# Jarvis73/BoxSegLiver

Hardware: AMD Instinct MI355X
Metric: CT slices/sec/node (fwd+bwd) UNet 256×256 bs=32; Dice vs ref (higher is better)
Workload: dtype f32

## Files before the change

### boxsegliver_amd/NetworksV2/UNet.py

```python
import torch

from .. import ops
from ..loss_metrics import build_head_desc, metrics_from_sums, pixel_weights
from ..utils import distribution_utils
from . import base
from .base import ModeKeys, ParamStore


def param_specs(in_channels, num_classes, init_channels, num_down_samples, normalizer, without_norm, name):
    specs = []

    def conv_unit(scope, cin, cout):
        specs.append((scope + "/weights", (3, 3, cin, cout), "conv_w"))
        if without_norm:
            specs.append((scope + "/biases", (cout,), "bias"))
        elif normalizer == "batch_norm":
            for leaf, kind in (("gamma", "gamma"), ("beta", "beta"), ("moving_mean", "moving_mean"),
                               ("moving_variance", "moving_var")):
                specs.append(("{}/BatchNorm/{}".format(scope, leaf), (cout,), kind))
        else:
            specs.append((scope + "/InstanceNorm/gamma", (cout,), "gamma"))
            specs.append((scope + "/InstanceNorm/beta", (cout,), "beta"))

    c, cin = init_channels, in_channels
# ... 33 lines not shown
        if self.params is not None:
            return
        in_ch = self.channel * (3 if getattr(self.args, "img_grad", False) else 1)
        specs = param_specs(in_ch, self.num_classes, init_channels, num_down_samples,
                            self.args.normalizer, getattr(self.args, "without_norm", False), self.name)
        self.params = ParamStore(specs, device, bias_decay=getattr(self.args, "bias_decay", False))
        self.params.initialize(self._get_initializer()[0], seed=getattr(self.args, "seed", None))

    def _net_arg_scope(self, *args, **kwargs):
        if getattr(self.args, "without_norm", False):
            self._norm = ("none", {})
        else:
            self._norm = self._get_normalization()
        return self._norm

    def _conv_unit(self, x, scope, out=None, pool=False):
        p = self.params
        kind, nparams = self._norm
        if kind == "none":
            spec = ops.NormSpec("none", 0.0, 0.0, self.is_training, self.compute_bf16)
            var = (None, p[scope + "/biases"], None, None)
        elif kind == "batch_norm":
            bn = scope + "/BatchNorm"
            spec = ops.NormSpec("batch_norm", nparams["eps"], nparams["decay"], bool(nparams["is_training"]),
                                self.compute_bf16)
            var = (p[bn + "/gamma"], p[bn + "/beta"], p[bn + "/moving_mean"], p[bn + "/moving_variance"])
        else:
            inn = scope + "/InstanceNorm"
            spec = ops.NormSpec("instance_norm", nparams["eps"], 0.0, self.is_training, self.compute_bf16)
            var = (p[inn + "/gamma"], p[inn + "/beta"], None, None)
        if pool:
            pooled, z = ops.Conv3x3NormReluPool.apply(x, p[scope + "/weights"], var[0], var[1], var[2], var[3], spec, out)
        else:
            z = ops.Conv3x3NormRelu.apply(x, p[scope + "/weights"], var[0], var[1], var[2], var[3], spec, out, None, None, None)
        if self._taps is not None:
            self._taps[scope] = z
        return (pooled, z) if pool else z

    def _build_network(self, *args, **kwargs):
        out_channels = kwargs.get("init_channels", 64)
        num_down_samples = kwargs.get("num_down_samples", 4)
        images = self._inputs["images"]
        if not images.is_cuda:
            raise ops._abi.UnetkError("UNet runs on the GPU only: move `images` to cuda (no CPU path)")
        if images.dim() != 4 or images.shape[3] != self.channel:
# ... 6 lines not shown
        nm = self.name

        if getattr(self.args, "img_grad", False):
            tensor_out = ops.image_gradients(images.to(torch.float32))
        else:
            tensor_out = images.contiguous()

        grad_mode = self.mode == ModeKeys.TRAIN
        with torch.set_grad_enabled(grad_mode):
            cats = {}
            skips = {}
            c = out_channels
            hh, ww = h, w
            for i in range(num_down_samples):
                s = "{}/Encode{}/Repeat/convolution2d_".format(nm, i + 1)
                tensor_out = self._conv_unit(tensor_out, s + "1")
                cat = torch.empty((n, hh, ww, 2 * c), dtype=self.storage_dtype, device=dev)
                skip_view = ops.alias(cat, 0, (n, hh, ww, c), cat.stride())
                tensor_out, skips[i] = self._conv_unit(tensor_out, s + "2", out=skip_view, pool=True)
                self._layers["Encode{:d}".format(i + 1)] = skips[i]
                cats[i] = cat
                c *= 2
                hh //= 2
                ww //= 2

            tensor_out = self._conv_unit(tensor_out, nm + "/ED-Bridge/ED-Bridge_1")
            tensor_out = self._conv_unit(tensor_out, nm + "/ED-Bridge/ED-Bridge_2")

            for i in reversed(range(num_down_samples)):
                c //= 2
                d = "{}/Decode{}".format(nm, i + 1)
                tensor_out = ops.DeconvConcat.apply(tensor_out, self.params[d + "/Conv2d_transpose/weights"],
                                                    self.params[d + "/Conv2d_transpose/biases"], skips[i], cats[i],
                                                    self.compute_bf16)
                tensor_out = self._conv_unit(tensor_out, d + "/Repeat/convolution2d_1")
                tensor_out = self._conv_unit(tensor_out, d + "/Repeat/convolution2d_2")

            self.ret_prob = kwargs.get("ret_prob", False)
            self.ret_pred = kwargs.get("ret_pred", False)
            labels = self._inputs.get("labels")
            if labels is not None:
                labels = labels.to(torch.int32).contiguous()
            pixel_w = pixel_weights(self.args, self._inputs, labels)
            desc = build_head_desc(self.args, n, h * w, c, self.num_classes,
                                   explicit_map=pixel_w is not None) if labels is not None else \
                ops.head_desc(n, h * w, c, self.num_classes)
            want_probs = bool(self.ret_prob or self.ret_pred or self.mode != ModeKeys.TRAIN)
            xent, dice, logits, probs, result = ops.HeadLoss.apply(
                tensor_out, self.params[nm + "/AdjustChannels/weights"], self.params[nm + "/AdjustChannels/biases"],
                labels, pixel_w, desc, want_probs)
# ... 42 lines not shown
```

### boxsegliver_amd/_abi.py

```python
import ctypes
import os
from ctypes import (POINTER, Structure, c_char_p, c_double, c_float, c_int, c_int32, c_int64, c_size_t,
                    c_void_p)

_LIB = None
LIB_PATH = os.environ.get("UNETK_LIB") or os.path.join(os.path.dirname(os.path.abspath(__file__)), "lib", "libunetk.so")

ABI_VERSION = 10
UNETK_MAX_CLASSES = 8
W_NONE, W_NUMERICAL, W_PROPORTION, W_PIXELMAP = 0, 1, 2, 3


class ConvDesc(Structure):
    _fields_ = [("N", c_int32), ("H", c_int32), ("W", c_int32), ("Cin", c_int32), ("Cout", c_int32),
                ("x_stride", c_int32), ("y_stride", c_int32), ("precision", c_int32), ("dilation", c_int32)]


FP32, BF16, BF16S = 0, 1, 2


class DeconvDesc(Structure):
    _fields_ = [("N", c_int32), ("H", c_int32), ("W", c_int32), ("Cin", c_int32), ("Cout", c_int32),
                ("out_stride", c_int32), ("out_coff", c_int32), ("precision", c_int32)]

# ... 30 lines not shown
class LitsGuideDesc(Structure):
    _fields_ = [("N", c_int32), ("H", c_int32), ("W", c_int32), ("C", c_int32), ("src_h", c_int32), ("src_w", c_int32),
                ("n_obj", c_int32), ("min_std", c_float)]


P = c_void_p
_SIGNATURES = {
    "unetk_lits_batch": (c_int, [POINTER(LitsDesc), c_void_p, c_void_p, c_void_p, c_void_p, c_void_p, c_void_p, c_void_p]),
    "unetk_lits_spatial_guide": (c_int, [POINTER(LitsGuideDesc), P, P, P, P, P]),
    "unetk_lits_context": (c_int, [P, c_int64, c_int, P, c_int, c_int, P, P, P, P]),
    "unetk_abi_version": (c_int, []),
    "unetk_nan_watch": (c_int, [P, P, c_int32, P]),
    "unetk_png_unfilter": (c_int, [P, c_int64, c_int, c_int, c_int, c_int, P, c_int64, P, P]),
    "unetk_conv3x3_fwd_affine_ok": (c_int, [POINTER(ConvDesc), c_int]),
    "unetk_conv3x3_fwd_affine": (c_int, [POINTER(ConvDesc), P, P, P, P, P, P, c_int, P, c_size_t, P]),
    "unetk_prof_reset": (c_int, [c_int]),
    "unetk_prof_enable": (c_int, [c_int]),
    "unetk_prof_mark": (c_int, []),
    "unetk_prof_read": (c_int, [c_int, c_int, POINTER(c_float)]),
    "unetk_prof_name": (c_int, [c_int, ctypes.c_char_p, c_int]),
    "unetk_error_string": (c_char_p, [c_int]),
    "unetk_conv3x3_pack": (c_int, [P, c_int, c_int, P, P, P]),
    "unetk_pack_item_blocks": (c_int, [c_int, c_int, c_int]),
    "unetk_pack_many": (c_int, [P, c_int, c_int, P]),
    "unetk_conv3x3_pack_bf16": (c_int, [P, c_int, c_int, P, P, P]),
    "unetk_conv3x3_pack_bf16s": (c_int, [P, c_int, c_int, P, P, P]),
    "unetk_conv3x3_stat_rows": (c_int, [POINTER(ConvDesc)]),
    "unetk_conv3x3_fwd": (c_int, [POINTER(ConvDesc), P, P, P, P, P]),
    "unetk_conv3x3_dgrad": (c_int, [POINTER(ConvDesc), P, P, P, P]),
    "unetk_conv3x3_ws_bytes": (c_size_t, [POINTER(ConvDesc)]),
# ... 136 lines not shown
```

### boxsegliver_amd/csrc/common.h

```cpp
#pragma once
#include <hip/hip_ext.h>
#include <hip/hip_runtime.h>
#include <stdint.h>

#include "unetk.h"

extern int g_unetk_prof_on;
void unetk_prof_pair(const void* fn, hipEvent_t* a, hipEvent_t* b);
#define UNETK_LAUNCH(kern, grid, block, lds, st, ...)                                                   \
  do {                                                                                                  \
    if (__builtin_expect(g_unetk_prof_on, 0)) {                                                         \
      hipEvent_t pa_, pb_;                                                                              \
      unetk_prof_pair(reinterpret_cast<const void*>(kern), &pa_, &pb_);                                 \
      hipExtLaunchKernelGGL(kern, grid, block, lds, st, pa_, pb_, 0, __VA_ARGS__);                      \
    } else {                                                                                            \
      hipLaunchKernelGGL(kern, grid, block, lds, st, __VA_ARGS__);                                      \
    }                                                                                                   \
  } while (0)

typedef float f32x16 __attribute__((ext_vector_type(16)));

#define UNETK_LAUNCH_CHECK()                      \
  do {                                            \
    hipError_t e_ = hipGetLastError();            \
// ... 97 lines not shown
  int stride;
  int Hin, Win, pbh, pbw;
  int ntaps[4], tap_off[4][4], tap_panel[4][4];
  int ooh[4], oow[4];
  int os, Hd, Wd;
  int dil;
  int kd, dshift0, dstep;
  int dsd, din;
  int64_t dplane;
  const void* ny;
  const float *nsc, *nsh, *nmu, *nrs;
  int nys, nsst;
  const float *asc, *ash;
  void* pool;
  int pool_s;
  float* sk_slab;
  size_t sk_slab_bytes;
  int sk_tiles, sk_nc, sk_maxp, sk_whole;
  int ng;
  int g_chan[12], g_dz[12], g_ntaps[12], g_off[12][4], g_panel[12][4];
  int dpar;
  int64_t dpar_yoff;
  int nlive;
  unsigned khalf;
  int klive[32];
};
inline int unetk_live_chunks(const uint32_t live8[2], int K) {
  const uint64_t m = (uint64_t)live8[0] | ((uint64_t)live8[1] << 32);
  if (m == 0 || K % 16 != 0 || K > 512) return K / 16;
  int n = 0;
// ... 78 lines not shown
```

### boxsegliver_amd/csrc/conv_igemm.hip

```cpp
#include "common.h"

#include <type_traits>
#include "pack.h"

namespace {

__device__ __attribute__((aligned(16))) float kZeroF4[4] = {};

constexpr int CK = 16;
#ifndef HALO_LD_T
#define HALO_LD_T 2
#endif
#ifndef HALO_ST_T
#define HALO_ST_T 7
#endif
constexpr int PS = 20;
constexpr int TW = 16;

#ifndef UNETK_HALO_ROWPAD
#define UNETK_HALO_ROWPAD 1
#endif
constexpr int halo_row_f(int S, int DIL) {
  return (S == 1 && DIL == 1 && UNETK_HALO_ROWPAD) ? ((S * TW + 2 * DIL) * PS + 63) / 64 * 64 : (S * TW + 2 * DIL) * PS;
}

template <int WM, int WN, int TM, int TN, int S = 1, int DIL = 1, int MODE = 0>
__global__ __launch_bounds__(WM* WN * 64, (TM * TN == 8 ? 2 : 1)) void conv3x3_igemm_kernel(ConvParams p) {
  constexpr bool NBR = MODE == 2, ACC = MODE == 1, AFF = MODE >= 3, POOL = MODE == 4;
  static_assert(!AFF || (S == 1 && DIL == 1), "the fused inference epilogue is for plain 3x3 convs");
  static_assert(S == 1 || DIL == 1, "strided atrous convs are not needed");
  static_assert(!NBR || (S == 1 && DIL == 1), "the fused reduction is for plain 3x3 convs");
  constexpr int NT = WM * WN * 64;
  constexpr int BM = WM * TM * 32, BN = WN * TN * 32;
  constexpr int TH = BM / TW, HH = S * TH + 2 * DIL;
  constexpr int HWD = S * TW + 2 * DIL;
  constexpr int HALO_PIX = HH * HWD;
  constexpr int HROW = halo_row_f(S, DIL);
  constexpr int HALO_F = HH * HROW;
  constexpr int WB_F = CK * BN;
  constexpr int HR = (HALO_PIX * 4 + NT - 1) / NT;
  constexpr int WR = (CK / 4 * BN + NT - 1) / NT;
  constexpr int WF4 = CK / 4 * BN;
  constexpr bool W_ALL = WF4 == WR * NT;

  extern __shared__ __attribute__((aligned(16))) float smem[];
  float* halo = smem;
  float* wbuf = smem + 2 * HALO_F;
// ... 5 lines not shown
  const int l31 = lane & 31, h = lane >> 5;

  const int bid = xcd_remap(blockIdx.x, gridDim.x);
  const int ntile = bid % p.n_ntiles;
  const int mtile = bid / p.n_ntiles;
  const int tw_i = mtile % p.tiles_w;
  const int th_i = (mtile / p.tiles_w) % p.tiles_h;
  const int n_img = mtile / (p.tiles_w * p.tiles_h);
  const int h0 = th_i * TH, w0 = tw_i * TW, n0 = ntile * BN;

  const int64_t ximg = p.xa.off(n_img), yimg = p.ya.off(n_img);

  int64_t hoff[HR];
  bool hok[HR];
  int hlds[HR];
#pragma unroll
  for (int r = 0; r < HR; ++r) {
    const int idx = tid + r * NT;
    const int pix = idx >> 2, q = idx & 3;
    const int hh = pix / HWD, ww = pix - hh * HWD;
    const int gh = S * h0 - (S == 1 ? DIL : p.pbh) + hh, gw = S * w0 - (S == 1 ? DIL : p.pbw) + ww;
    const int Hin = S == 1 ? p.H : p.Hin, Win = S == 1 ? p.W : p.Win;
    hok[r] = (idx < HALO_PIX * 4) && gh >= 0 && gh < Hin && gw >= 0 && gw < Win;
    hoff[r] = ximg + ((int64_t)gh * Win + gw) * p.xs + q * 4;
    hlds[r] = (idx < HALO_PIX * 4) ? hh * HROW + ww * PS + q * 4 : -1;
  }
  const int cin4 = p.Cin >> 2;
  int64_t woff[WR];
#pragma unroll
  for (int r = 0; r < WR; ++r) {
    const int idx = min(tid + r * NT, WF4 - 1);
    const int q = idx / BN, n = idx - q * BN;
    woff[r] = ((int64_t)q * p.Cout + n0 + n) * 4;
  }

  const int nchunks = p.Cin / CK;
  int c_begin = 0, c_end = nchunks;
  if (p.kd > 1) {
    const int dep = n_img % p.spg;
    int dt_lo = 0, dt_hi = p.kd;
    while (dt_lo < dt_hi && dep * p.dsd + p.dshift0 + dt_lo < 0) ++dt_lo;
    while (dt_hi > dt_lo && dep * p.dsd + p.dshift0 + dt_hi - 1 >= p.din) --dt_hi;
    c_begin = dt_lo * nchunks;
    c_end = dt_hi * nchunks;
  }
  float4 hreg[HR], wreg[WR];
  auto load_halo = [&](int cc) {
    const int dt = p.kd > 1 ? cc / nchunks : 0, c = cc - dt * nchunks;
    const int64_t soff = (p.kd > 1 ? (int64_t)(p.dshift0 + dt) * p.dplane : 0) + c * CK;
#pragma unroll
    for (int r = 0; r < HR; ++r) hreg[r] = ldg4(hok[r] ? p.x + hoff[r] + soff : kZeroF4);
  };
  auto store_halo = [&](int buf) {
#pragma unroll
    for (int r = 0; r < HR; ++r)
      if (hlds[r] >= 0) *reinterpret_cast<float4*>(&halo[buf * HALO_F + hlds[r]]) = hreg[r];
  };
  auto load_w = [&](int cc, int t) {
    const int dt = p.kd > 1 ? cc / nchunks : 0, c = cc - dt * nchunks;
    const float* base = p.wp + ((int64_t)(dt * 9 + t) * cin4 + c * (CK / 4)) * p.Cout * 4;
#pragma unroll
    for (int r = 0; r < WR; ++r)
      wreg[r] = ldg4(base + woff[r]);
  };
  auto store_w = [&](int buf) {
#pragma unroll
    for (int r = 0; r < WR; ++r)
      if (W_ALL || tid + r * NT < WF4) *reinterpret_cast<float4*>(&wbuf[buf * WB_F + (tid + r * NT) * 4]) = wreg[r];
// ... 5 lines not shown
    const int sub = wm * TM + tm;
    abase[tm] = S * (2 * sub + (l31 >> 4)) * HROW + S * (l31 & 15) * PS + 4 * h;
  }
  const int bbase = (h * BN + wn * TN * 32 + l31) * 4;

  f32x16 acc[TM][TN];
#pragma unroll
  for (int tm = 0; tm < TM; ++tm)
#pragma unroll
    for (int tn = 0; tn < TN; ++tn)
#pragma unroll
      for (int r = 0; r < 16; ++r) acc[tm][tn][r] = 0.f;

  load_halo(c_begin);
  load_w(c_begin, 0);
  store_halo(0);
  store_w(0);
  __syncthreads();

  int step = 0;
  for (int c = c_begin; c < c_end; ++c) {
    const float* hb = halo + ((c - c_begin) & 1) * HALO_F;
    const bool more_chunks = (c + 1 < c_end);
#pragma unroll
    for (int t = 0; t < 9; ++t, ++step) {
      const bool has_next = (t < 8) || more_chunks;
      if (has_next) load_w(t < 8 ? c : c + 1, t < 8 ? t + 1 : 0);
      if (t == HALO_LD_T && more_chunks) load_halo(c + 1);
      __builtin_amdgcn_sched_barrier(0);

      const float* wb = wbuf + (step & 1) * WB_F;
      const int toff = (t / 3) * DIL * HROW + (t % 3) * DIL * PS;
#pragma unroll
      for (int g = 0; g < CK / 8; ++g) {
        float4 a[TM], b[TN];
#pragma unroll
        for (int tm = 0; tm < TM; ++tm)
          a[tm] = *reinterpret_cast<const float4*>(&hb[abase[tm] + toff + 8 * g]);
#pragma unroll
        for (int tn = 0; tn < TN; ++tn)
          b[tn] = *reinterpret_cast<const float4*>(&wb[bbase + (2 * g * BN + tn * 32) * 4]);
#pragma unroll
        for (int tm = 0; tm < TM; ++tm)
#pragma unroll
          for (int tn = 0; tn < TN; ++tn) {
            acc[tm][tn] = __builtin_amdgcn_mfma_f32_32x32x2f32(a[tm].x, b[tn].x, acc[tm][tn], 0, 0, 0);
            acc[tm][tn] = __builtin_amdgcn_mfma_f32_32x32x2f32(a[tm].y, b[tn].y, acc[tm][tn], 0, 0, 0);
            acc[tm][tn] = __builtin_amdgcn_mfma_f32_32x32x2f32(a[tm].z, b[tn].z, acc[tm][tn], 0, 0, 0);
            acc[tm][tn] = __builtin_amdgcn_mfma_f32_32x32x2f32(a[tm].w, b[tn].w, acc[tm][tn], 0, 0, 0);
          }
      }

      if (has_next) store_w((step + 1) & 1);
      if (t == HALO_ST_T && more_chunks) store_halo((c + 1 - c_begin) & 1);
      __syncthreads();
    }
  }

  float ssum[TN], ssq[TN];
#pragma unroll
  for (int tn = 0; tn < TN; ++tn) ssum[tn] = ssq[tn] = 0.f;
  float nsc[TN], nsh[TN], nmu[TN], nrs[TN];
  if constexpr (NBR) {
#pragma unroll
    for (int tn = 0; tn < TN; ++tn) {
      const int64_t o = (int64_t)n_img * p.nsst + n0 + (wn * TN + tn) * 32 + l31;
      nsc[tn] = p.nsc[o]; nsh[tn] = p.nsh[o]; nmu[tn] = p.nmu[o]; nrs[tn] = p.nrs[o];
    }
  }
// ... 372 lines not shown
  static bool attr_done = false;
  if (!attr_done) {
    hipError_t e = hipFuncSetAttribute((const void*)kern, hipFuncAttributeMaxDynamicSharedMemorySize, (int)lds);
    if (e != hipSuccess) return (int)e;
    attr_done = true;
  }
  const int grid = n_mtiles * p.n_ntiles;
  UNETK_LAUNCH(kern, dim3(grid), dim3(WM * WN * 64), lds, st, p);
  UNETK_LAUNCH_CHECK();
  return UNETK_OK;
}

template <int WM, int WN, int TM, int TN, int S = 1, int DIL = 1, bool NBR = false>
int launch_igemm(const ConvParams& p, int n_mtiles, hipStream_t st) {
  if constexpr (NBR) return launch_igemm_mode<WM, WN, TM, TN, S, DIL, 2>(p, n_mtiles, st);
  if (p.asc != nullptr) {
    if constexpr (S == 1 && DIL == 1) {
      if (p.accumulate || p.stat != nullptr) return UNETK_E_UNSUPPORTED;
      return p.pool != nullptr ? launch_igemm_mode<WM, WN, TM, TN, 1, 1, 4>(p, n_mtiles, st)
                               : launch_igemm_mode<WM, WN, TM, TN, 1, 1, 3>(p, n_mtiles, st);
    } else {
      return UNETK_E_UNSUPPORTED;
    }
  }
  if (p.accumulate) return launch_igemm_mode<WM, WN, TM, TN, S, DIL, 1>(p, n_mtiles, st);
  return launch_igemm_mode<WM, WN, TM, TN, S, DIL, 0>(p, n_mtiles, st);
}

}

static int s2_th(int Cout) { return Cout % 128 == 0 ? 4 : 8; }
int unetk_conv_stat_rows(int N, int H, int W, int Cin, int Cout, int spg, int stride, int dil) {
  if (dil == 2) return N * ((H + 7) / 8) * ((W + TW - 1) / TW);
  if (stride == 2) return N * ((H + s2_th(Cout) - 1) / s2_th(Cout)) * ((W + TW - 1) / TW);
  if (unetk_conv_lin_ok(N, H, W, Cin, Cout, spg)) return unetk_conv_stat_rows_lin(N, H, W, spg, Cout);
  const int th = tile_rows(N, H, W, Cin, Cout, spg, false);
  return N * ((H + th - 1) / th) * ((W + TW - 1) / TW);
}

bool unetk_conv_stride2_ok(int Cin, int Cout) { return Cin % CK == 0 && Cout % 64 == 0; }

int unetk_conv_run(ConvParams p, hipStream_t st) {
  if ((p.ny != nullptr || p.asc != nullptr) && (p.stride == 2 || p.dil == 2)) return UNETK_E_UNSUPPORTED;
  if (p.stride == 2) {
    if (p.bf16 || !unetk_conv_stride2_ok(p.Cin, p.Cout) || p.xs % 4 != 0) return UNETK_E_UNSUPPORTED;
    p.tiles_h = (p.H + s2_th(p.Cout) - 1) / s2_th(p.Cout);
    p.tiles_w = (p.W + TW - 1) / TW;
    const int n_mt = p.N * p.tiles_h * p.tiles_w;
    p.stat_rows = n_mt;
    if (p.Cout % 128 == 0) {
      p.n_ntiles = p.Cout / 128;
      return launch_igemm<2, 2, 1, 2, 2>(p, n_mt, st);
    }
    p.n_ntiles = p.Cout / 64;
    return launch_igemm<4, 1, 1, 2, 2>(p, n_mt, st);
  }
  if (p.dil == 2) {
    if (p.bf16 || p.Cin % CK != 0 || p.Cout % 64 != 0 || p.xs % 4 != 0) return UNETK_E_UNSUPPORTED;
// ... 190 lines not shown
  ConvParams p{};
  if (d->precision == UNETK_BF16S) {
    if (unetk_conv_bf16_ok(d->Cin, d->Cout)) p.bf16 = UNETK_BF16S;
    else p.ybf16 = 1;
  }
  p.x = (const float*)x; p.wp = (const float*)w; p.y = (float*)z; p.stat = nullptr;
  p.asc = scale; p.ash = shift; p.pool = pooled; p.pool_s = pooled_stride;
  if (ws && unetk_aligned16(ws) && ws_bytes > 0) { p.sk_slab = (float*)ws; p.sk_slab_bytes = ws_bytes; }
  p.dil = d->dilation;
  p.N = d->N; p.H = d->H; p.W = d->W; p.Cin = d->Cin; p.Cout = d->Cout; p.xs = d->x_stride; p.ys = d->y_stride;
  p.xa = unetk_dense_addr(p.H, p.W, p.xs);
  p.ya = unetk_dense_addr(p.H, p.W, p.ys);
  return unetk_conv_run(p, (hipStream_t)stream);
}

extern "C" int unetk_conv3x3_dgrad(const unetk_conv_desc* d, const void* dy, const void* w, void* dx,
                                   void* stream) {
  return unetk_conv3x3_dgrad_ws(d, dy, w, dx, nullptr, 0, stream);
}

extern "C" int unetk_conv3x3_dgrad_ws(const unetk_conv_desc* d, const void* dy, const void* w, void* dx, void* ws,
                                      size_t ws_bytes, void* stream) {
  UNETK_REQUIRE(conv_desc_ok(d) && dy && w && dx);
  UNETK_REQUIRE(unetk_aligned16(dy) && unetk_aligned16(w) && unetk_aligned16(dx));
  if (pick_cfg(d->Cout, d->Cin).id < 0) return UNETK_E_UNSUPPORTED;
  UNETK_REQUIRE(d->x_stride % 4 == 0 && d->y_stride % 4 == 0);
  if (d->precision != UNETK_FP32 && !unetk_conv_bf16_ok(d->Cout, d->Cin)) return UNETK_E_UNSUPPORTED;
  if (d->precision == UNETK_BF16S && d->dilation > 1) return UNETK_E_UNSUPPORTED;
  ConvParams p{};
  p.bf16 = d->precision;
// ... 44 lines not shown
```

### boxsegliver_amd/ops.py

```python
import ctypes
import os

import torch

from . import _abi
from ._abi import Conv3dDesc, ConvDesc, Deconv3dDesc, DeconvDesc, HeadDesc, NormDesc, check, ptr, stream_ptr


class _Workspace(object):

    def __init__(self):
        self._bufs = {}

    def get(self, nbytes, device):
        nbytes = max(int(nbytes), 16)
        key = (device.type, device.index)
        buf = self._bufs.get(key)
        if buf is None or buf.numel() < nbytes:
            buf = torch.empty(int(nbytes * 1.25) + 256, dtype=torch.uint8, device=device)
            self._bufs[key] = buf
        return buf


WORKSPACE = _Workspace()
FUSE_EVAL = os.environ.get("UNETK_FUSE_EVAL", "1") != "0"
FUSE_NBR = True
FUSED_NBR = {}
DEBUG_CAPTURE = None
PROFILE_SHAPES = False
PROFILE = None


PACK_BATCH = True
PARAM_GEN = 0
_PARAM_FLATS = {}


def register_param_buffer(flat):
    import weakref
    _PARAM_FLATS[flat.untyped_storage().data_ptr()] = weakref.ref(flat)

# ... 131 lines not shown


def _timed(tag_fn, flops, fmt=None, args=(), nbytes_fn=None):
    if PROFILE is None:
        return _NO_TIMER
    tag = tag_fn() if callable(tag_fn) else tag_fn
    return _Timed(tag, flops, fmt.format(*args) if fmt else None, nbytes_fn(tag) if nbytes_fn else 0)


def _timed_hbm(tag, t, passes, extra=0):
    if PROFILE is None:
        return _NO_TIMER
    return _Timed(tag, 0.0, None, t.numel() * t.element_size() * passes + extra)


def _igemm_tag(cin, cout, bf16=False, h=0, n=1 << 20, w=1 << 10, nbr=False):
    def cdiv(a, b):
        return -(-a // b)

    def big(bn):
        return h % 16 == 0 and not (nbr and cin < 256) and n * (h // 16) * cdiv(w, 16) * (cout // bn) >= 512
    if bf16 and cin % 32 == 0 and cout % 32 == 0:
        bs = ",true>" if int(bf16) == _abi.BF16S else ">"
        if int(bf16) == _abi.BF16S and h >= 24 and (cout % 128 == 0 or cout == 64):
            bn = 128 if cout % 128 == 0 else 64
            if n * cdiv(h, 32) * cdiv(w, 16) * (cout // bn) >= 200:
                return "conv3x3_bf16s_kernel<{}{}>".format(bn // 16, ",nbr" if nbr else "")
        if cout % 128 == 0:
            tall = h >= 24 and n * cdiv(h, 32) * cdiv(w, 16) * (cout // 128) >= 200
            return ("conv3x3_igemm_bf16_kernel<4,2,4,2" if tall else "conv3x3_igemm_bf16_kernel<2,2,2,2") + bs
        if cout % 64 == 0:
# ... 202 lines not shown
                      "conv3x3_pack_bf16")
            kind, perm = PK_CONV_BF16, 1 if prec == _abi.BF16S else 0
        else:
            wp_f = torch.empty(9 * cin * cout, dtype=torch.float32, device=w.device)
            wp_d = torch.empty_like(wp_f) if want_dgrad else None
            check(_abi.lib().unetk_conv3x3_pack(ptr(w), cin, cout, ptr(wp_f), ptr(wp_d), stream_ptr()), "conv3x3_pack")
            kind, perm = PK_CONV_F32, 0
        return wp_f, wp_d, [(kind, perm, cin, cout, w.data_ptr(), wp_f.data_ptr(), wp_d.data_ptr() if want_dgrad else None)]
    return PACKS.get(w, ("c3", prec, bool(want_dgrad)), build)


def conv_uses_mfma(cin, cout):
    return cin % 16 == 0 and cout % 32 == 0


def conv3x3_fwd(x, w, cout, want_stats=True, y=None, bf16=False, dilation=1):
    _require_cuda(x, w)
    n, h, wd, cin = x.shape
    prec = precision_of(bf16)
    if y is None:
        y = torch.empty((n, h, wd, cout), dtype=storage_dtype(prec), device=x.device)
    if prec == _abi.BF16S:
        assert y.dtype == torch.bfloat16 and x.dtype == (torch.bfloat16 if conv_uses_mfma(cin, cout) else torch.float32), \
            (x.dtype, y.dtype, cin, cout)
    else:
        assert x.dtype == torch.float32 and y.dtype == torch.float32
    d = ConvDesc(n, h, wd, cin, cout, _pix_stride(x), _pix_stride(y), prec, int(dilation))
    stats = None
    rows = 0
    if want_stats:
        rows = _abi.lib().unetk_conv3x3_stat_rows(ctypes.byref(d))
        if rows <= 0:
            check(rows, "conv3x3_stat_rows")
        stats = torch.empty((2, rows, cout), dtype=torch.float32, device=x.device)
    nws = _abi.lib().unetk_conv3x3_ws_bytes(ctypes.byref(d)) if prec == _abi.FP32 else 0
    ws = WORKSPACE.get(nws, x.device) if nws else None
    with _timed(lambda: _igemm_tag(cin, cout, bf16, h, n, wd), 18.0 * n * h * wd * cin * cout, "fwd {}x{}x{} {}->{}", (n, h, wd, cin, cout),
                lambda tag: (x.numel() * x.element_size() + y.numel() * y.element_size()) if tag in ("conv3x3_direct_kernel", "conv3x3_c3_mfma_kernel") else 0):
        check(_abi.lib().unetk_conv3x3_fwd_ws(ctypes.byref(d), ptr(x), ptr(w), ptr(y), ptr(stats), ptr(ws), nws,
                                              stream_ptr()), "conv3x3_fwd")
    return y, stats, rows


def conv3x3_fwd_affine(x, w, cout, scale, shift, z=None, pool=False, bf16=False):
    _require_cuda(x, w)
    n, h, wd, cin = x.shape
    prec = precision_of(bf16)
    if z is None:
        z = torch.empty((n, h, wd, cout), dtype=storage_dtype(prec), device=x.device)
    d = ConvDesc(n, h, wd, cin, cout, _pix_stride(x), _pix_stride(z), prec, 1)
    pooled = torch.empty((n, h // 2, wd // 2, cout), dtype=z.dtype, device=x.device) if pool else None
# ... 928 lines not shown
    check(_abi.lib().unetk_norm_se_bwd_add(ctypes.byref(d), ptr(y), ptr(dy), ptr(aff[0]), ptr(aff[1]), ptr(aff[2]),
                                           ptr(a_mat.contiguous()), ptr(k2.contiguous()), stream_ptr()), "norm_se_bwd_add")
    return dy


class NormSpec(object):

    def __init__(self, kind="batch_norm", eps=1e-3, decay=0.999, training=True, bf16=False):
        assert kind in ("batch_norm", "instance_norm", "none")
        self.kind, self.eps, self.decay, self.training = kind, eps, decay, training
        self.guide_leaky = False
        self.guide_alpha = 0.2
        self.guide_per_sample = False
        self.guide_post = False
        self.dropout = None
        self.se = None
        self.bf16 = precision_of(bf16)

    @property
    def per_sample(self):
        return self.kind == "instance_norm"


class Conv3x3NormRelu(_Op):

    @staticmethod
    def forward(ctx, x, w, gamma, beta, moving_mean, moving_var, spec, out, guide, gw, gb, den=None, dilation=1, se_feat=None):
        _require_cuda(x, w)
        cin, cout = w.shape[2], w.shape[3]
        dilation = int(dilation or 1)
        if dilation != 1 and (bool(getattr(spec, "bf16", False)) or not conv_uses_mfma(cin, cout)):
            raise _abi.UnetkError("atrous conv (rate {}) needs the fp32 MFMA path (Cin % 16, Cout % 64)".format(dilation))
        if den is not None:
            den = den.contiguous()
        mfma = conv_uses_mfma(cin, cout)
        prec = precision_of(getattr(spec, "bf16", 0))
        bf16 = prec if conv_uses_bf16(cin, cout) else 0
        if prec == _abi.BF16S:
            if mfma and (cin % 64 or cout % 64):
                raise _abi.UnetkError("bf16 storage needs Cin % 64 == 0 and Cout % 64 == 0 (got {}->{})".format(cin, cout))
            bf16 = prec
        need_dx = ctx.needs_input_grad[0]
        if mfma:
            wp_f, wp_d = conv3x3_pack(w, want_dgrad=need_dx, bf16=bf16)
        else:
            wp_f, wp_d = w, None
            if need_dx:
                raise _abi.UnetkError("conv3x3 input gradient needs Cin%64==0 and Cout%16==0 "
                                      "(got {}->{})".format(cin, cout))
        plain = spec.kind == "none"
        se = getattr(spec, "se", None)
        use_batch_stats = (spec.training or spec.per_sample) and not plain
        if se is not None and (plain or den is not None):
            raise _abi.UnetkError("--use_se needs a normalised unit and no other density gain")
        fprec = precision_of(bf16)
        if FUSE_EVAL and not spec.training and not use_batch_stats and se is None and den is None and guide is None \
                and gb is None and fprec in (_abi.FP32, _abi.BF16S) and dilation == 1:
# ... 6 lines not shown
                nd = norm_desc((n_, h_, w_, cout), False, _pix_stride(z), 0, 0, 0)
                if plain:
                    sc, sh = torch.ones_like(beta), beta.detach().contiguous()
                else:
                    aff = norm_finalize(nd, None, 0, gamma, beta, spec.eps, spec.decay, False, moving_mean, moving_var, x.device)
                    sc, sh = aff[2], aff[3]
                pooled = torch.empty((n_, h_ // 2, w_ // 2, cout), dtype=z.dtype, device=x.device) if with_pool else None
                tag = _igemm_tag(cin, cout, bf16, h_, n_, w_) + ("+affine+relu+pool" if with_pool else "+affine+relu")
                nws = _abi.lib().unetk_conv3x3_ws_bytes(ctypes.byref(fd))
                ws = WORKSPACE.get(nws, x.device) if nws else None
                with _timed(tag, 18.0 * n_ * h_ * w_ * cin * cout, "infer {}x{}x{} {}->{}", (n_, h_, w_, cin, cout)):
                    check(_abi.lib().unetk_conv3x3_fwd_affine(ctypes.byref(fd), ptr(x), ptr(wp_f), ptr(sc), ptr(sh), ptr(z),
                                                              ptr(pooled), cout, ptr(ws), nws, stream_ptr()), "conv3x3_fwd_affine")
                ctx.pooled = pooled
                return alias(z) if out is not None else z
        y, stats, rows = conv3x3_fwd(x, wp_f, cout, want_stats=use_batch_stats or se is not None, bf16=bf16, dilation=dilation)
        z = out if out is not None else torch.empty_like(y)
        g_ch = 0 if guide is None else guide.shape[-1]
        if g_ch:
            gw = gw.contiguous()
        if gb is not None:
            gb = gb.contiguous()
        d = norm_desc(y.shape, spec.per_sample, _pix_stride(z), g_ch, cout if g_ch else 0, 0)
        if g_ch and getattr(spec, "guide_leaky", False):
            alpha = float(getattr(spec, "guide_alpha", 0.2))
            d.guide_leaky = 1 if alpha == 0.2 else 2
            d.guide_alpha = alpha
        if g_ch and getattr(spec, "guide_post", False):
            d.guide_leaky = 3
        if getattr(spec, "guide_per_sample", False):
            d.guide_per_sample = 1
# ... 21 lines not shown
                mean_b = norm_finalize(ps, stats, rows, None, None, spec.eps, 0.0, True, None, None, y.device)[0]
                xhat_mean = ((mean_b - aff[0]) * aff[1]).detach()
            with torch.enable_grad():
                g_leaf = gamma.detach().requires_grad_(True) if gamma is not None else None
                b_leaf = beta.detach().requires_grad_(True) if beta is not None else None
                pooled = xhat_mean if g_leaf is None else xhat_mean * g_leaf
                if b_leaf is not None:
                    pooled = pooled + (b_leaf if m_mean is None else m_mean * b_leaf)
                pooled = pooled + torch.zeros_like(xhat_mean).requires_grad_(True) if not pooled.requires_grad else pooled
                pooled.retain_grad()
                f_leaf = se_feat.detach().requires_grad_(True) if se_feat is not None else None
                gains = se(pooled, f_leaf)
            den = gains.detach().contiguous()
            se_graph = (g_leaf, b_leaf, pooled, gains, xhat_mean, f_leaf, m_mean)
        ctx.pooled = None
        if getattr(ctx, "want_pool", False) and POOL_FUSED and se is None and den is None and g_ch == 0 and gb is None \
                and d.dropout_keep == 0 and y.shape[1] % 2 == 0 and y.shape[2] % 2 == 0:
            ctx.pooled = norm_apply_relu_pool(d, y, aff, z)
        else:
            norm_apply_relu(d, y, aff, z, guide, gw, gb, den)
        simple = (not plain and se is None and den is None and g_ch == 0 and gb is None and d.dropout_keep == 0)
        if spec.training:
            src = getattr(x, "_unetk_unit", None)
            ctx.producer = src if (need_dx and src is not None and dilation == 1) else None
            ctx.simple = simple
            if getattr(ctx, "want_pool", False):
                ctx.unit_saved = (x, y, aff, guide, gw, gb, den)
            else:
                ctx.save_for_backward(x, y, aff, guide, gw, gb, den)
            ctx.se_graph = se_graph
            ctx.wp_d = wp_d
            ctx.need_dx = need_dx
            ctx.bf16 = bf16
            ctx.dilation = dilation
            ctx.desc = d
            ctx.has = (gamma is not None, beta is not None)
            ctx.sinks = (grad_sink(w, ctx), grad_sink(gamma, ctx) if se is None else None, grad_sink(beta, ctx) if se is None and not plain else None)
            ctx.w_dbg = w.detach() if DEBUG_CAPTURE is not None else None
            ctx.gb_dbg = (gamma, beta) if DEBUG_CAPTURE is not None else None
            ctx.z_dbg = z.detach() if DEBUG_CAPTURE is not None else None
        zr = alias(z) if out is not None else z
        if spec.training and simple and out is None:
            zr._unetk_unit = (y, aff, spec.per_sample)
        return zr

    @staticmethod
    def backward(ctx, dz):
        return Conv3x3NormRelu._backward(ctx, dz)

    @staticmethod
    def _backward(ctx, dz, pool=None):
        x, y, aff, guide, gw, gb, den = ctx.saved_tensors[:7]
        pre = None
        if pool is None:
            pre = FUSED_NBR.pop(dz.data_ptr(), None) if DEBUG_CAPTURE is None else None
            if pre is not None and not (ctx.simple and pre[0] == y.data_ptr() and pre[1] == tuple(dz.shape) and dz.is_contiguous()
                                        and pre[4] == dz._version):
                pre = None
# ... 419 lines not shown
```

### include/unetk.h

```cpp
#ifndef UNETK_H_
#define UNETK_H_

#include <stddef.h>
#include <stdint.h>

#ifdef __cplusplus
extern "C" {
#endif

#define UNETK_OK 0
#define UNETK_E_BADARG (-1)
#define UNETK_E_UNSUPPORTED (-2)
#define UNETK_E_WORKSPACE (-3)

#define UNETK_MAX_CLASSES 8

#define UNETK_W_NONE 0
#define UNETK_W_NUMERICAL 1
#define UNETK_W_PROPORTION 2
#define UNETK_W_PIXELMAP 3

#define UNETK_LOSS_XENTROPY 1
#define UNETK_LOSS_DICE 2

// ... 40 lines not shown
                      float* stat_partials, void* stream);

int unetk_conv3x3_dgrad(const unetk_conv_desc* d, const void* dy, const void* w, void* dx,
                        void* stream);

size_t unetk_conv3x3_ws_bytes(const unetk_conv_desc* d);
int unetk_conv3x3_fwd_ws(const unetk_conv_desc* d, const void* x, const void* w, void* y, float* stat_partials,
                         void* ws, size_t ws_bytes, void* stream);
int unetk_conv3x3_dgrad_ws(const unetk_conv_desc* d, const void* dy, const void* w, void* dx, void* ws,
                           size_t ws_bytes, void* stream);

int unetk_conv3x3_fwd_affine_ok(const unetk_conv_desc* d, int with_pool);
int unetk_conv3x3_fwd_affine(const unetk_conv_desc* d, const void* x, const void* w, const float* scale,
                             const float* shift, void* z, void* pooled, int pooled_stride, void* ws, size_t ws_bytes,
                             void* stream);

int unetk_conv3x3_dgrad_nbr_rows(const unetk_conv_desc* d);
int unetk_conv3x3_dgrad_nbr(const unetk_conv_desc* d, const void* dy, const void* w, void* dx, const void* prod_y,
                            int prod_y_stride, const float* scale, const float* shift, const float* mean,
                            const float* rstd, int per_sample, float* partials, void* stream);

size_t unetk_conv3x3_wgrad_ws_bytes(const unetk_conv_desc* d);
int unetk_conv3x3_wgrad(const unetk_conv_desc* d, const void* x, const void* dy, float* dw,
                        void* ws, size_t ws_bytes, void* stream);

typedef struct unetk_conv3d_desc {
  int32_t N, D, H, W, Cin, Cout;
  int32_t kd;
  int32_t sd;
  int32_t shw;
// ... 252 lines not shown
```

Before: 437.5.

## Fold norm+ReLU of first conv into next conv's halo loader

```diff
diff --git a/boxsegliver_amd/NetworksV2/UNet.py b/boxsegliver_amd/NetworksV2/UNet.py
--- a/boxsegliver_amd/NetworksV2/UNet.py
+++ b/boxsegliver_amd/NetworksV2/UNet.py
@@ -71,7 +71,7 @@
             self._norm = self._get_normalization()
         return self._norm
 
-    def _conv_unit(self, x, scope, out=None, pool=False):
+    def _conv_unit(self, x, scope, out=None, pool=False, defer=False):
         p = self.params
         kind, nparams = self._norm
         if kind == "none":
@@ -86,6 +86,7 @@
             inn = scope + "/InstanceNorm"
             spec = ops.NormSpec("instance_norm", nparams["eps"], 0.0, self.is_training, self.compute_bf16)
             var = (p[inn + "/gamma"], p[inn + "/beta"], None, None)
+        spec.defer_apply = bool(defer) and not pool and self._taps is None
         if pool:
             pooled, z = ops.Conv3x3NormReluPool.apply(x, p[scope + "/weights"], var[0], var[1], var[2], var[3], spec, out)
         else:
@@ -122,7 +123,7 @@
             hh, ww = h, w
             for i in range(num_down_samples):
                 s = "{}/Encode{}/Repeat/convolution2d_".format(nm, i + 1)
-                tensor_out = self._conv_unit(tensor_out, s + "1")
+                tensor_out = self._conv_unit(tensor_out, s + "1", defer=True)
                 cat = torch.empty((n, hh, ww, 2 * c), dtype=self.storage_dtype, device=dev)
                 skip_view = ops.alias(cat, 0, (n, hh, ww, c), cat.stride())
                 tensor_out, skips[i] = self._conv_unit(tensor_out, s + "2", out=skip_view, pool=True)
@@ -132,7 +133,7 @@
                 hh //= 2
                 ww //= 2
 
-            tensor_out = self._conv_unit(tensor_out, nm + "/ED-Bridge/ED-Bridge_1")
+            tensor_out = self._conv_unit(tensor_out, nm + "/ED-Bridge/ED-Bridge_1", defer=True)
             tensor_out = self._conv_unit(tensor_out, nm + "/ED-Bridge/ED-Bridge_2")
 
             for i in reversed(range(num_down_samples)):
@@ -141,7 +142,7 @@
                 tensor_out = ops.DeconvConcat.apply(tensor_out, self.params[d + "/Conv2d_transpose/weights"],
                                                     self.params[d + "/Conv2d_transpose/biases"], skips[i], cats[i],
                                                     self.compute_bf16)
-                tensor_out = self._conv_unit(tensor_out, d + "/Repeat/convolution2d_1")
+                tensor_out = self._conv_unit(tensor_out, d + "/Repeat/convolution2d_1", defer=True)
                 tensor_out = self._conv_unit(tensor_out, d + "/Repeat/convolution2d_2")
 
             self.ret_prob = kwargs.get("ret_prob", False)
diff --git a/boxsegliver_amd/_abi.py b/boxsegliver_amd/_abi.py
--- a/boxsegliver_amd/_abi.py
+++ b/boxsegliver_amd/_abi.py
@@ -68,6 +68,8 @@
     "unetk_png_unfilter": (c_int, [P, c_int64, c_int, c_int, c_int, c_int, P, c_int64, P, P]),
     "unetk_conv3x3_fwd_affine_ok": (c_int, [POINTER(ConvDesc), c_int]),
     "unetk_conv3x3_fwd_affine": (c_int, [POINTER(ConvDesc), P, P, P, P, P, P, c_int, P, c_size_t, P]),
+    "unetk_conv3x3_fwd_apply_ok": (c_int, [POINTER(ConvDesc)]),
+    "unetk_conv3x3_fwd_apply": (c_int, [POINTER(ConvDesc), P, P, P, c_int, P, P, P, P, P]),
     "unetk_prof_reset": (c_int, [c_int]),
     "unetk_prof_enable": (c_int, [c_int]),
     "unetk_prof_mark": (c_int, []),
diff --git a/boxsegliver_amd/csrc/common.h b/boxsegliver_amd/csrc/common.h
--- a/boxsegliver_amd/csrc/common.h
+++ b/boxsegliver_amd/csrc/common.h
@@ -135,6 +135,9 @@
   const float *asc, *ash;
   void* pool;
   int pool_s;
+  const float *lsc, *lsh;
+  float* lz;
+  int lsst;
   float* sk_slab;
   size_t sk_slab_bytes;
   int sk_tiles, sk_nc, sk_maxp, sk_whole;
diff --git a/boxsegliver_amd/csrc/conv_igemm.hip b/boxsegliver_amd/csrc/conv_igemm.hip
--- a/boxsegliver_amd/csrc/conv_igemm.hip
+++ b/boxsegliver_amd/csrc/conv_igemm.hip
@@ -26,11 +26,13 @@
 
 template <int WM, int WN, int TM, int TN, int S = 1, int DIL = 1, int MODE = 0>
 __global__ __launch_bounds__(WM* WN * 64, (TM * TN == 8 ? 2 : 1)) void conv3x3_igemm_kernel(ConvParams p) {
-  constexpr bool NBR = MODE == 2, ACC = MODE == 1, AFF = MODE >= 3, POOL = MODE == 4;
+  constexpr bool NBR = MODE == 2, ACC = MODE == 1, AFF = MODE == 3 || MODE == 4, POOL = MODE == 4, APL = MODE == 5;
+  static_assert(!APL || (S == 1 && DIL == 1), "the normaliser in the loader is for plain 3x3 convs");
   static_assert(!AFF || (S == 1 && DIL == 1), "the fused inference epilogue is for plain 3x3 convs");
   static_assert(S == 1 || DIL == 1, "strided atrous convs are not needed");
   static_assert(!NBR || (S == 1 && DIL == 1), "the fused reduction is for plain 3x3 convs");
   constexpr int NT = WM * WN * 64;
+  static_assert(NT % 4 == 0, "a thread's halo slots share one channel quad");
   constexpr int BM = WM * TM * 32, BN = WN * TN * 32;
   constexpr int TH = BM / TW, HH = S * TH + 2 * DIL;
   constexpr int HWD = S * TW + 2 * DIL;
@@ -66,6 +68,7 @@
   int64_t hoff[HR];
   bool hok[HR];
   int hlds[HR];
+  bool hzo[APL ? HR : 1];
 #pragma unroll
   for (int r = 0; r < HR; ++r) {
     const int idx = tid + r * NT;
@@ -76,6 +79,7 @@
     hok[r] = (idx < HALO_PIX * 4) && gh >= 0 && gh < Hin && gw >= 0 && gw < Win;
     hoff[r] = ximg + ((int64_t)gh * Win + gw) * p.xs + q * 4;
     hlds[r] = (idx < HALO_PIX * 4) ? hh * HROW + ww * PS + q * 4 : -1;
+    if constexpr (APL) hzo[r] = hok[r] && ntile == 0 && hh >= DIL && hh < HH - DIL && ww >= DIL && ww < HWD - DIL;
   }
   const int cin4 = p.Cin >> 2;
   int64_t woff[WR];
@@ -97,13 +101,40 @@
     c_end = dt_hi * nchunks;
   }
   float4 hreg[HR], wreg[WR];
+  float4 lsc = make_float4(0.f, 0.f, 0.f, 0.f), lsh = lsc;
+  const float* lsc_p = nullptr;
+  const float* lsh_p = nullptr;
+  if constexpr (APL) {
+    lsc_p = p.lsc + (int64_t)n_img * p.lsst + (tid & 3) * 4;
+    lsh_p = p.lsh + (int64_t)n_img * p.lsst + (tid & 3) * 4;
+  }
   auto load_halo = [&](int cc) {
     const int dt = p.kd > 1 ? cc / nchunks : 0, c = cc - dt * nchunks;
     const int64_t soff = (p.kd > 1 ? (int64_t)(p.dshift0 + dt) * p.dplane : 0) + c * CK;
 #pragma unroll
     for (int r = 0; r < HR; ++r) hreg[r] = ldg4(hok[r] ? p.x + hoff[r] + soff : kZeroF4);
+    if constexpr (APL) {
+      lsc = ldg4(lsc_p + c * CK);
+      lsh = ldg4(lsh_p + c * CK);
+    }
   };
-  auto store_halo = [&](int buf) {
+  auto store_halo = [&](int buf, int cc) {
+    if constexpr (APL) {
+      const float4 sh = make_float4(lsh.x + 0.f, lsh.y + 0.f, lsh.z + 0.f, lsh.w + 0.f);
+#pragma unroll
+      for (int r = 0; r < HR; ++r) {
+        float4 u;
+        u.x = fmaxf(fmaf(hreg[r].x, lsc.x, sh.x), 0.f); u.y = fmaxf(fmaf(hreg[r].y, lsc.y, sh.y), 0.f);
+        u.z = fmaxf(fmaf(hreg[r].z, lsc.z, sh.z), 0.f); u.w = fmaxf(fmaf(hreg[r].w, lsc.w, sh.w), 0.f);
+        if (!hok[r]) u = make_float4(0.f, 0.f, 0.f, 0.f);
+        hreg[r] = u;
+        if (hlds[r] >= 0) *reinterpret_cast<float4*>(&halo[buf * HALO_F + hlds[r]]) = u;
+      }
+#pragma unroll
+      for (int r = 0; r < HR; ++r)
+        if (hzo[r]) stg4(p.lz + hoff[r] + cc * CK, hreg[r]);
+      return;
+    }
 #pragma unroll
     for (int r = 0; r < HR; ++r)
       if (hlds[r] >= 0) *reinterpret_cast<float4*>(&halo[buf * HALO_F + hlds[r]]) = hreg[r];
@@ -139,7 +170,7 @@
 
   load_halo(c_begin);
   load_w(c_begin, 0);
-  store_halo(0);
+  store_halo(0, c_begin);
   store_w(0);
   __syncthreads();
 
@@ -149,8 +180,8 @@
     const bool more_chunks = (c + 1 < c_end);
 #pragma unroll
     for (int t = 0; t < 9; ++t, ++step) {
-      const bool has_next = (t < 8) || more_chunks;
-      if (has_next) load_w(t < 8 ? c : c + 1, t < 8 ? t + 1 : 0);
+      const bool has_next = APL || (t < 8) || more_chunks;
+      if (has_next) load_w((t < 8 || !more_chunks) ? c : c + 1, t < 8 ? t + 1 : 0);
       if (t == HALO_LD_T && more_chunks) load_halo(c + 1);
       __builtin_amdgcn_sched_barrier(0);
 
@@ -176,8 +207,9 @@
           }
       }
 
+      if constexpr (APL) __builtin_amdgcn_sched_barrier(0);
       if (has_next) store_w((step + 1) & 1);
-      if (t == HALO_ST_T && more_chunks) store_halo((c + 1 - c_begin) & 1);
+      if (t == HALO_ST_T && more_chunks) store_halo((c + 1 - c_begin) & 1, c + 1);
       __syncthreads();
     }
   }
@@ -580,6 +612,14 @@
 template <int WM, int WN, int TM, int TN, int S = 1, int DIL = 1, bool NBR = false>
 int launch_igemm(const ConvParams& p, int n_mtiles, hipStream_t st) {
   if constexpr (NBR) return launch_igemm_mode<WM, WN, TM, TN, S, DIL, 2>(p, n_mtiles, st);
+  if (p.lz != nullptr) {
+    if constexpr (S == 1 && DIL == 1) {
+      if (p.accumulate || p.asc != nullptr || p.kd > 1) return UNETK_E_UNSUPPORTED;
+      return launch_igemm_mode<WM, WN, TM, TN, 1, 1, 5>(p, n_mtiles, st);
+    } else {
+      return UNETK_E_UNSUPPORTED;
+    }
+  }
   if (p.asc != nullptr) {
     if constexpr (S == 1 && DIL == 1) {
       if (p.accumulate || p.stat != nullptr) return UNETK_E_UNSUPPORTED;
@@ -607,7 +647,10 @@
 bool unetk_conv_stride2_ok(int Cin, int Cout) { return Cin % CK == 0 && Cout % 64 == 0; }
 
 int unetk_conv_run(ConvParams p, hipStream_t st) {
-  if ((p.ny != nullptr || p.asc != nullptr) && (p.stride == 2 || p.dil == 2)) return UNETK_E_UNSUPPORTED;
+  if ((p.ny != nullptr || p.asc != nullptr || p.lz != nullptr) && (p.stride == 2 || p.dil == 2)) return UNETK_E_UNSUPPORTED;
+  if (p.lz != nullptr && (p.bf16 || p.ny != nullptr || pick_cfg(p.Cin, p.Cout).id < 0 ||
+                          unetk_conv_lin_ok(p.N, p.H, p.W, p.Cin, p.Cout, p.spg < 1 ? 1 : p.spg)))
+    return UNETK_E_UNSUPPORTED;
   if (p.stride == 2) {
     if (p.bf16 || !unetk_conv_stride2_ok(p.Cin, p.Cout) || p.xs % 4 != 0) return UNETK_E_UNSUPPORTED;
     p.tiles_h = (p.H + s2_th(p.Cout) - 1) / s2_th(p.Cout);
@@ -828,6 +871,29 @@
   return unetk_conv_run(p, (hipStream_t)stream);
 }
 
+extern "C" int unetk_conv3x3_fwd_apply_ok(const unetk_conv_desc* d) {
+  if (!conv_desc_ok(d) || d->dilation > 1 || d->precision != UNETK_FP32) return 0;
+  if (pick_cfg(d->Cin, d->Cout).id < 0 || d->x_stride != d->Cin || d->y_stride % 4 != 0) return 0;
+  return unetk_conv_lin_ok(d->N, d->H, d->W, d->Cin, d->Cout, 1) ? 0 : 1;
+}
+
+extern "C" int unetk_conv3x3_fwd_apply(const unetk_conv_desc* d, const void* prod_y, const float* scale, const float* shift,
+                                       int per_sample, void* z, const void* w, void* y, float* stat_partials,
+                                       void* stream) {
+  UNETK_REQUIRE(conv_desc_ok(d) && prod_y && scale && shift && z && w && y);
+  UNETK_REQUIRE(unetk_aligned16(prod_y) && unetk_aligned16(z) && unetk_aligned16(w) && unetk_aligned16(y));
+  UNETK_REQUIRE(unetk_aligned16(scale) && unetk_aligned16(shift));
+  if (!unetk_conv3x3_fwd_apply_ok(d)) return UNETK_E_UNSUPPORTED;
+  ConvParams p{};
+  p.x = (const float*)prod_y; p.wp = (const float*)w; p.y = (float*)y; p.stat = stat_partials;
+  p.lsc = scale; p.lsh = shift; p.lz = (float*)z; p.lsst = per_sample ? d->Cin : 0;
+  p.dil = d->dilation;
+  p.N = d->N; p.H = d->H; p.W = d->W; p.Cin = d->Cin; p.Cout = d->Cout; p.xs = d->x_stride; p.ys = d->y_stride;
+  p.xa = unetk_dense_addr(p.H, p.W, p.xs);
+  p.ya = unetk_dense_addr(p.H, p.W, p.ys);
+  return unetk_conv_run(p, (hipStream_t)stream);
+}
+
 extern "C" int unetk_conv3x3_dgrad(const unetk_conv_desc* d, const void* dy, const void* w, void* dx,
                                    void* stream) {
   return unetk_conv3x3_dgrad_ws(d, dy, w, dx, nullptr, 0, stream);
diff --git a/boxsegliver_amd/ops.py b/boxsegliver_amd/ops.py
--- a/boxsegliver_amd/ops.py
+++ b/boxsegliver_amd/ops.py
@@ -25,6 +25,7 @@
 WORKSPACE = _Workspace()
 FUSE_EVAL = os.environ.get("UNETK_FUSE_EVAL", "1") != "0"
 FUSE_NBR = True
+APPLY_IN_LOADER = os.environ.get("UNETK_APPLY_IN_LOADER", "1") != "0"
 FUSED_NBR = {}
 DEBUG_CAPTURE = None
 PROFILE_SHAPES = False
@@ -186,7 +187,9 @@
     return _Timed(tag, 0.0, None, t.numel() * t.element_size() * passes + extra)
 
 
-def _igemm_tag(cin, cout, bf16=False, h=0, n=1 << 20, w=1 << 10, nbr=False):
+def _igemm_tag(cin, cout, bf16=False, h=0, n=1 << 20, w=1 << 10, nbr=False, apply=False):
+    if apply:
+        return _igemm_tag(cin, cout, bf16, h, n, w, nbr) + "+apply"
     def cdiv(a, b):
         return -(-a // b)
 
@@ -419,7 +422,24 @@
     return cin % 16 == 0 and cout % 32 == 0
 
 
-def conv3x3_fwd(x, w, cout, want_stats=True, y=None, bf16=False, dilation=1):
+def conv3x3_fwd_apply_ok(x, cout, bf16=False, dilation=1):
+    n, h, wd, cin = x.shape
+    if precision_of(bf16) != _abi.FP32 or int(dilation) != 1 or x.dtype != torch.float32 or not x.is_contiguous():
+        return False
+    d = ConvDesc(n, h, wd, cin, cout, cin, cout, _abi.FP32, 1)
+    return _abi.lib().unetk_conv3x3_fwd_apply_ok(ctypes.byref(d)) == 1
+
+
+def materialize(z):
+    pend = getattr(z, "_unetk_deferred", None)
+    if pend is not None:
+        z._unetk_deferred = None
+        py, paff, _, nd = pend
+        norm_apply_relu(nd, py, paff, z)
+    return z
+
+
+def conv3x3_fwd(x, w, cout, want_stats=True, y=None, bf16=False, dilation=1, deferred=None):
     _require_cuda(x, w)
     n, h, wd, cin = x.shape
     prec = precision_of(bf16)
@@ -440,6 +460,14 @@
         stats = torch.empty((2, rows, cout), dtype=torch.float32, device=x.device)
     nws = _abi.lib().unetk_conv3x3_ws_bytes(ctypes.byref(d)) if prec == _abi.FP32 else 0
     ws = WORKSPACE.get(nws, x.device) if nws else None
+    if deferred is not None:
+        py, paff, per_sample = deferred[0], deferred[1], deferred[2]
+        assert py.is_contiguous() and x.is_contiguous() and tuple(py.shape) == tuple(x.shape) and py.dtype == x.dtype == torch.float32
+        with _timed(lambda: _igemm_tag(cin, cout, bf16, h, n, wd, apply=True), 18.0 * n * h * wd * cin * cout, "fwd+apply {}x{}x{} {}->{}",
+                    (n, h, wd, cin, cout)):
+            check(_abi.lib().unetk_conv3x3_fwd_apply(ctypes.byref(d), ptr(py), ptr(paff[2]), ptr(paff[3]), 1 if per_sample else 0,
+                                                     ptr(x), ptr(w), ptr(y), ptr(stats), stream_ptr()), "conv3x3_fwd_apply")
+        return y, stats, rows
     with _timed(lambda: _igemm_tag(cin, cout, bf16, h, n, wd), 18.0 * n * h * wd * cin * cout, "fwd {}x{}x{} {}->{}", (n, h, wd, cin, cout),
                 lambda tag: (x.numel() * x.element_size() + y.numel() * y.element_size()) if tag in ("conv3x3_direct_kernel", "conv3x3_c3_mfma_kernel") else 0):
         check(_abi.lib().unetk_conv3x3_fwd_ws(ctypes.byref(d), ptr(x), ptr(w), ptr(y), ptr(stats), ptr(ws), nws,
@@ -1398,6 +1426,7 @@
         self.guide_per_sample = False
         self.guide_post = False
         self.dropout = None
+        self.defer_apply = False
         self.se = None
         self.bf16 = precision_of(bf16)
 
@@ -1425,6 +1454,13 @@
                 raise _abi.UnetkError("bf16 storage needs Cin % 64 == 0 and Cout % 64 == 0 (got {}->{})".format(cin, cout))
             bf16 = prec
         need_dx = ctx.needs_input_grad[0]
+        deferred = getattr(x, "_unetk_deferred", None)
+        if deferred is not None:
+            if APPLY_IN_LOADER and spec.training and mfma and not bf16 and conv3x3_fwd_apply_ok(x, cout, bf16, dilation):
+                x._unetk_deferred = None
+            else:
+                materialize(x)
+                deferred = None
         if mfma:
             wp_f, wp_d = conv3x3_pack(w, want_dgrad=need_dx, bf16=bf16)
         else:
@@ -1461,7 +1497,8 @@
                                                               ptr(pooled), cout, ptr(ws), nws, stream_ptr()), "conv3x3_fwd_affine")
                 ctx.pooled = pooled
                 return alias(z) if out is not None else z
-        y, stats, rows = conv3x3_fwd(x, wp_f, cout, want_stats=use_batch_stats or se is not None, bf16=bf16, dilation=dilation)
+        y, stats, rows = conv3x3_fwd(x, wp_f, cout, want_stats=use_batch_stats or se is not None, bf16=bf16, dilation=dilation,
+                                     deferred=deferred)
         z = out if out is not None else torch.empty_like(y)
         g_ch = 0 if guide is None else guide.shape[-1]
         if g_ch:
@@ -1513,12 +1550,16 @@
             den = gains.detach().contiguous()
             se_graph = (g_leaf, b_leaf, pooled, gains, xhat_mean, f_leaf, m_mean)
         ctx.pooled = None
-        if getattr(ctx, "want_pool", False) and POOL_FUSED and se is None and den is None and g_ch == 0 and gb is None \
+        simple = (not plain and se is None and den is None and g_ch == 0 and gb is None and d.dropout_keep == 0)
+        defer = (APPLY_IN_LOADER and bool(getattr(spec, "defer_apply", False)) and spec.training and simple and out is None
+                 and not getattr(ctx, "want_pool", False) and y.dtype == torch.float32 and y.is_contiguous())
+        if defer:
+            pass
+        elif getattr(ctx, "want_pool", False) and POOL_FUSED and se is None and den is None and g_ch == 0 and gb is None \
                 and d.dropout_keep == 0 and y.shape[1] % 2 == 0 and y.shape[2] % 2 == 0:
             ctx.pooled = norm_apply_relu_pool(d, y, aff, z)
         else:
             norm_apply_relu(d, y, aff, z, guide, gw, gb, den)
-        simple = (not plain and se is None and den is None and g_ch == 0 and gb is None and d.dropout_keep == 0)
         if spec.training:
             src = getattr(x, "_unetk_unit", None)
             ctx.producer = src if (need_dx and src is not None and dilation == 1) else None
@@ -1541,6 +1582,8 @@
         zr = alias(z) if out is not None else z
         if spec.training and simple and out is None:
             zr._unetk_unit = (y, aff, spec.per_sample)
+        if defer:
+            zr._unetk_deferred = (y, aff, spec.per_sample, d)
         return zr
 
     @staticmethod
diff --git a/include/unetk.h b/include/unetk.h
--- a/include/unetk.h
+++ b/include/unetk.h
@@ -78,6 +78,10 @@
 int unetk_conv3x3_fwd_affine(const unetk_conv_desc* d, const void* x, const void* w, const float* scale,
                              const float* shift, void* z, void* pooled, int pooled_stride, void* ws, size_t ws_bytes,
                              void* stream);
+
+int unetk_conv3x3_fwd_apply_ok(const unetk_conv_desc* d);
+int unetk_conv3x3_fwd_apply(const unetk_conv_desc* d, const void* prod_y, const float* scale, const float* shift,
+                            int per_sample, void* z, const void* w, void* y, float* stat_partials, void* stream);
 
 int unetk_conv3x3_dgrad_nbr_rows(const unetk_conv_desc* d);
 int unetk_conv3x3_dgrad_nbr(const unetk_conv_desc* d, const void* dy, const void* w, void* dx, const void* prod_y,
```

New measurement: 440.2, median of 6. No clear change (+0.6%).
